# zypher-game/uzkge

Hardware: AMD Instinct MI355X
Metric: bn254_g1_msm_points_per_sec (higher is better)
Workload: dtype u256 (254-bit modular integers: 8 x u32 Montgomery limbs in HBM, 9 x 29-bit limbs in the two hot loops); 1 GPU; BN254 G1 MSM, 2^24 random points + uniform scalars per GPU, bases resident in HBM; points_per_gpu=16777216, total_points=16777216

## Files before the change

### uzkge_amd/csrc/api.cpp

```cpp
#include <algorithm>
#include <atomic>
#include <cstdarg>
#include <cstdlib>
#include <cstring>
#include <exception>
#include <new>

#include "ctx.hpp"
#include "host_ec64.hpp"
#include "host_math.hpp"

namespace uzk {

static thread_local char g_err[512] = "";

void set_error(const char* fmt, ...) {
    va_list ap;
    va_start(ap, fmt);
    vsnprintf(g_err, sizeof g_err, fmt, ap);
    va_end(ap);
}

int on_exception(const char* fn) noexcept {
    try { throw; }
// ... 270 lines not shown
        if (kv.second.owned && kv.second.d_points) (void)hipFree(kv.second.d_points);
        if (kv.second.d_table) (void)hipFree(kv.second.d_table);
    }
    s.srs.clear();
    s.num_cus.clear();
    s.bound = false;
    s.device = -1;
    return UZK_OK;
} catch (...) { return uzk::on_exception("uzk_shutdown"); }

namespace uzk {
static void copy_tuning(const Ctx& from, Ctx& to) {
    to.msm_window_bits = from.msm_window_bits;
    to.tune_no_precompute = from.tune_no_precompute; to.tune_ntt_tile = from.tune_ntt_tile; to.tune_ntt_two_pass = from.tune_ntt_two_pass; to.tune_small = from.tune_small;
    to.tune_chunk_log = from.tune_chunk_log; to.tune_stream_log = from.tune_stream_log; to.tune_stream_min_log = from.tune_stream_min_log;
    to.tune_seg_sort = from.tune_seg_sort; to.tune_arith29 = from.tune_arith29;
}
}
int uzk_ctx_create(uint64_t* ctx_out) try {
    if (!ctx_out) { set_error("uzk_ctx_create: null pointer"); return UZK_ERR_PARAMETER; }
    Ctx* c = new Ctx();
    {
        API_LOCK;
        int rc = require_ready();
        if (rc != UZK_OK) { delete c; return rc; }
        copy_tuning(ctx(), *c);
    }
    Shared& s = shared();
    std::lock_guard<std::mutex> lk(s.mu);
    const uint64_t h = s.next_ctx++;
    s.contexts[h] = c;
// ... 937 lines not shown
    if (!window_bits || !windows || n == 0) { set_error("uzk_msm_plan_info: bad arguments"); return UZK_ERR_PARAMETER; }
    msm_plan_info(ctx(), n, window_bits, windows);
    return UZK_OK;
} catch (...) { return uzk::on_exception("uzk_msm_plan_info"); }

int uzk_tune(const char* key, int value) try {
    API_LOCK;
    if (!key) { set_error("uzk_tune: null key"); return UZK_ERR_PARAMETER; }
    Ctx& c = ctx();
    if (!std::strcmp(key, "msm_no_precompute")) c.tune_no_precompute = value;
    else if (!std::strcmp(key, "msm_stream_log")) c.tune_stream_log = (value >= -1 && value <= 26) ? value : 0;
    else if (!std::strcmp(key, "msm_stream_min_log")) c.tune_stream_min_log = (value >= 4 && value <= 26) ? value : 22;
    else if (!std::strcmp(key, "msm_chunk_log")) c.tune_chunk_log = (value >= 8 && value <= 26) ? value : 26;
    else if (!std::strcmp(key, "msm_small")) c.tune_small = value ? 1 : 0;
    else if (!std::strcmp(key, "msm_seg_sort")) c.tune_seg_sort = value;
    else if (!std::strcmp(key, "ntt_tile")) c.tune_ntt_tile = (value == 1024 || value == 2048) ? value : 0;
    else if (!std::strcmp(key, "ntt_two_pass")) c.tune_ntt_two_pass = value ? 1 : 0;
    else if (!std::strcmp(key, "arith29")) c.tune_arith29 = value & 7;
    else { set_error("uzk_tune: unknown key %s", key); return UZK_ERR_PARAMETER; }
    return UZK_OK;
} catch (...) { return uzk::on_exception("uzk_tune"); }

}
```

### uzkge_amd/csrc/ctx.hpp

```cpp
#pragma once
#include <hip/hip_runtime.h>

#include <cstdint>
#include <cstdlib>
#include <cstdio>
#include <chrono>
#include <map>
#include <mutex>
#include <string>
#include <vector>

#include "../../include/uzkge_gpu.h"
#include "../../include/uzkge_gpu_test.h"
#include "ec.hpp"

namespace uzk {

void set_error(const char* fmt, ...);
int on_exception(const char* fn) noexcept;

#define UZK_HIP(expr)                                                                      \
    do {                                                                                   \
        hipError_t _e = (expr);                                                            \
        if (_e != hipSuccess) {                                                            \
// ... 63 lines not shown
    Fp* msm_tail_host = nullptr;
    size_t msm_tail_cap = 0;
    int msm_window_bits = 0;
    int tune_no_precompute = 0;
    int tune_ntt_two_pass = 1;
    int tune_ntt_tile = 0;
    int tune_small = 1;
    int tune_chunk_log = 26;
    int tune_stream_log = 0;
    int tune_stream_min_log = 22;
    int tune_arith29 = default_arith29();
    static int default_arith29() {
        static const int v = [] { const char* e = std::getenv("UZK_ARITH29"); return e ? std::atoi(e) : 7; }();
        return v;
    }
    int tune_seg_sort = 1;
    DevBuf poly_tmp, poly_tmp2, poly_io, zpoly_tmp, open_tmp, poly_args;
    DevBuf poly_cnt;
    uint32_t trim_flip = 0;
    void* poly_host = nullptr;
    size_t poly_host_cap = 0;
    DevBuf ntt_sub;
    struct PowCache { Fp key; bool valid = false; uint64_t stamp = 0; DevBuf buf; };
    PowCache pow_cache[8];
    uint64_t pow_stamp = 0;
    std::vector<void*> ntt_fused;
    std::map<uint64_t, void*> g1ntt_plans;
    DevBuf g1ntt_work, g1ntt_prefix, g1ntt_io;
    struct Srs {
        Affine* d_points = nullptr;
// ... 151 lines not shown
```

### uzkge_amd/csrc/msm.hip

```cpp
#include <algorithm>
#include <cmath>
#include <mutex>
#include <functional>
#include <memory>
#include <condition_variable>
#include <atomic>
#include <cstring>
#include <thread>
#include <vector>

#include "ctx.hpp"
#include "ec29.hpp"
#include "ecquad.hpp"
#include "ecquad29.hpp"
#include "ec29l.hpp"
#include "host_ec64.hpp"
#include "host_math.hpp"

namespace uzk {

constexpr uint32_t kSeg = 16;
constexpr uint32_t kSignBit = 0x80000000u;
constexpr uint32_t kCombineFan = 32;
constexpr int kMaxPasses = 3;
// ... 485 lines not shown
            }
        }
        __syncthreads();
        if (!direct) {
            const uint32_t hl = tid & 31;
            for (uint32_t b = b_lo + (tid >> 5); b < b_hi; b += TB / 32) {
                const uint32_t c = cnt[b], src = off[b] - base, dst = gdst[b];
                for (uint32_t j = hl; j < c; j += 32) out[dst + j] = buf[src + j];
            }
            __syncthreads();
        }
        b_lo = b_hi;
    }
}

__global__ __launch_bounds__(1024) void msm_scan_win_kernel(const uint32_t* __restrict__ cnt_in, uint32_t div,
                                                            uint32_t* __restrict__ v_out,
                                                            uint32_t* __restrict__ off_out,
                                                            uint32_t* __restrict__ win_total,
                                                            uint32_t* __restrict__ max_out, uint32_t NB,
                                                            uint32_t* __restrict__ len_hist = nullptr) {
    __shared__ uint32_t part[1024];
    __shared__ uint32_t lh[256];
    extern __shared__ uint32_t stage[];
    if (len_hist != nullptr) { if (threadIdx.x < 256) lh[threadIdx.x] = 0; __syncthreads(); }
    const uint32_t w = blockIdx.x, tid = threadIdx.x;
    const uint32_t per = (NB + 1023) / 1024;
    const uint32_t lo = min(NB, tid * per), hi = min(NB, lo + per);
    const uint32_t* cnt = cnt_in + (size_t)w * NB;
    const uint64_t magic = div ? ((1ull << 40) + div - 1) / div : 0;
    const bool fast = div && div <= 1024;
    auto val = [&](uint32_t c) -> uint32_t {
        if (!div) return c;
        if (fast && c < (1u << 29)) return (uint32_t)(((uint64_t)(c + div - 1) * magic) >> 40);
        return (c + div - 1) / div;
    };
    auto pad = [](uint32_t i) -> uint32_t { return i + (i >> 5); };
    uint32_t mx = 0;
    for (uint32_t i = tid; i < NB; i += 1024) {
        const uint32_t c = cnt[i];
        mx = max(mx, c);
        const uint32_t T = val(c);
        stage[pad(i)] = T;
        if (len_hist != nullptr && c != 0) {
            const uint32_t q = c / T, r = c - q * T;
            if (r) atomicAdd(&lh[min(q + 1, 255u)], r);
            atomicAdd(&lh[min(q, 255u)], T - r);
        }
    }
    __syncthreads();
    if (len_hist != nullptr && tid < 256 && lh[tid]) atomicAdd(&len_hist[tid], lh[tid]);
    uint32_t s = 0;
    for (uint32_t b = lo; b < hi; ++b) s += stage[pad(b)];
    part[tid] = s;
    __syncthreads();
    for (uint32_t off = 1; off < 1024; off <<= 1) {
        uint32_t v = (tid >= off) ? part[tid - off] : 0;
        __syncthreads();
        part[tid] += v;
        __syncthreads();
    }
    uint32_t run = part[tid] - s;
    for (uint32_t b = lo; b < hi; ++b) {
        const uint32_t v = stage[pad(b)];
        stage[pad(b)] = run;
        run += v;
    }
    __syncthreads();
    uint32_t* off_o = off_out + (size_t)w * NB;
    uint32_t* v_o = v_out ? v_out + (size_t)w * NB : nullptr;
    for (uint32_t i = tid; i < NB; i += 1024) {
        off_o[i] = stage[pad(i)];
        if (v_o) v_o[i] = val(cnt[i]);
    }
    if (tid == 1023) win_total[w] = part[1023];
    if (max_out) {
        for (int o = 32; o > 0; o >>= 1) mx = max(mx, (uint32_t)__shfl_down((int)mx, o));
        if ((tid & 63) == 0 && mx) atomicMax(max_out, mx);
    }
}
static size_t scan_win_lds(uint32_t NB) {
    static const bool raised = [] {
        return hipFuncSetAttribute(reinterpret_cast<const void*>(msm_scan_win_kernel), hipFuncAttributeMaxDynamicSharedMemorySize,
                                   ((1 << 15) + (1 << 10) + 1) * 4) == hipSuccess;
    }();
    (void)raised;
    return ((size_t)NB + NB / 32 + 1) * 4;
}
__global__ __launch_bounds__(1024) void msm_win_base_kernel(const uint32_t* __restrict__ win_total,
                                                            uint32_t* __restrict__ win_base, uint32_t W) {
    __shared__ uint32_t part[1024];
    const uint32_t tid = threadIdx.x;
    const uint32_t v = tid < W ? win_total[tid] : 0;
// ... 22 lines not shown
        if (win_base[mid] <= tid) lo = mid; else hi = mid;
    }
    w = lo;
    const uint32_t lt = tid - win_base[w];
    const uint32_t* off = task_off + (size_t)w * NB;
    lo = 0; hi = NB;
    while (hi - lo > 1) {
        const uint32_t mid = (lo + hi) >> 1;
        if (off[mid] <= lt) lo = mid; else hi = mid;
    }
    b = lo;
    j = lt - off[lo];
}

struct TaskDesc { uint32_t start, cnt, task; uint32_t pad; };
constexpr uint32_t kLenBins = 256;

__global__ __launch_bounds__(256) void msm_task_scan_kernel(const uint32_t* __restrict__ hist, uint32_t* __restrict__ cursor) {
    __shared__ uint32_t h[kLenBins];
    h[threadIdx.x] = hist[threadIdx.x];
    __syncthreads();
    if (threadIdx.x == 0) {
        uint32_t run = 0;
        for (int l = kLenBins - 1; l >= 0; --l) { const uint32_t v = h[l]; h[l] = run; run += v; }
    }
    __syncthreads();
    cursor[threadIdx.x] = h[threadIdx.x];
}
constexpr uint32_t kFillInline = 4;
struct BigBucket { uint32_t start, total, T, tid0; };
__global__ __launch_bounds__(256) void msm_bucket_fill_kernel(const uint32_t* __restrict__ win_base, const uint32_t* __restrict__ task_cnt,
                                                              const uint32_t* __restrict__ task_off,
                                                              const uint32_t* __restrict__ bucket_start,
                                                              const uint32_t* __restrict__ bucket_count, uint32_t NB, uint64_t TBK,
                                                              uint32_t* __restrict__ cursor, TaskDesc* __restrict__ desc,
                                                              uint32_t* __restrict__ big_count, BigBucket* __restrict__ big, uint32_t direct) {
    __shared__ uint32_t h[kLenBins], base[kLenBins];
    h[threadIdx.x] = 0;
    __syncthreads();
    const uint64_t t = (uint64_t)blockIdx.x * blockDim.x + threadIdx.x;
    uint32_t T = 0, total = 0, q = 0, r = 0, start = 0, tid0 = 0, rank_hi = 0, rank_lo = 0;
    bool inline_fill = false;
    if (t < TBK) {
        T = task_cnt[t];
        if (T != 0) {
            total = bucket_count[t];
            start = bucket_start[t];
            tid0 = win_base[t / NB] + task_off[t];
            q = total / T; r = total - q * T;
            if (T <= kFillInline) {
                inline_fill = true;
                if (r) rank_hi = atomicAdd(&h[min(q + 1, kLenBins - 1)], r);
                rank_lo = atomicAdd(&h[min(q, kLenBins - 1)], T - r);
            } else {
                BigBucket e; e.start = start; e.total = total; e.T = T; e.tid0 = tid0;
                big[atomicAdd(big_count, 1u)] = e;
            }
        }
    }
    __syncthreads();
    if (h[threadIdx.x]) base[threadIdx.x] = atomicAdd(&cursor[threadIdx.x], h[threadIdx.x]);
    __syncthreads();
    if (inline_fill) {
        const uint32_t p_hi = base[min(q + 1, kLenBins - 1)] + rank_hi, p_lo = base[min(q, kLenBins - 1)] + rank_lo;
        for (uint32_t j = 0; j < T; ++j) {
            TaskDesc d;
            d.start = start + j * q + min(j, r);
            d.cnt = q + (j < r ? 1u : 0u);
            d.task = (direct && T == 1) ? (kSignBit | (uint32_t)t) : tid0 + j;
            d.pad = 0;
            desc[j < r ? p_hi + j : p_lo + (j - r)] = d;
        }
    }
}
__global__ __launch_bounds__(64) void msm_task_fill_big_kernel(const uint32_t* __restrict__ big_count, const BigBucket* __restrict__ big,
                                                               uint32_t* __restrict__ cursor, TaskDesc* __restrict__ desc) {
// ... 101 lines not shown
    for (int o = GS / 2; o > 0; o >>= 1) {
        XYZZ q = xyzz_shfl_down(acc, o);
        if (sub + (uint32_t)o < (uint32_t)GS) xyzz_add(acc, q);
    }
    return acc;
}

struct BigFold { uint32_t src, cnt, dst, pad; };
template <int GS>
__global__ __launch_bounds__(256) void msm_combine_kernel(const XYZZ* __restrict__ in, const uint32_t* __restrict__ in_cnt,
                                                          const uint32_t* __restrict__ in_off,
                                                          const uint32_t* __restrict__ in_base,
                                                          const uint32_t* __restrict__ task_off,
                                                          const uint32_t* __restrict__ win_base, XYZZ* __restrict__ out,
                                                          uint32_t NB, uint32_t W, uint32_t G, uint32_t* __restrict__ big_count,
                                                          BigFold* __restrict__ big, uint32_t big_thresh, int arith29) {
    const uint32_t gt = blockIdx.x * blockDim.x + threadIdx.x;
    const uint32_t tid = gt / GS, sub = gt % GS;
    if (tid >= win_base[W]) return;
    uint32_t w, b, j;
    find_task(tid, win_base, W, task_off, NB, w, b, j);
    const uint32_t total = in_cnt[(size_t)w * NB + b];
    const uint32_t first = j * G;
    const uint32_t cnt = min(G, total - first);
    const uint32_t at = in_base[w] + in_off[(size_t)w * NB + b] + first;
    if (GS == 1 && big != nullptr && cnt > big_thresh) {
        BigFold e; e.src = at; e.cnt = cnt; e.dst = tid; e.pad = 0;
        big[atomicAdd(big_count, 1u)] = e;
        return;
    }
    XYZZ acc = arith29 ? fold_partials29<GS>(in + at, cnt, sub) : fold_partials<GS>(in + at, cnt, sub);
    if (sub == 0) out[tid] = acc;
}
__global__ __launch_bounds__(64) void msm_fold_big_kernel(const XYZZ* __restrict__ in, const uint32_t* __restrict__ big_count,
                                                          const BigFold* __restrict__ big, XYZZ* __restrict__ out, int accumulate) {
    const uint32_t total = *big_count, lane = threadIdx.x;
    for (uint32_t i = blockIdx.x; i < total; i += gridDim.x) {
        const BigFold e = big[i];
        XYZZ acc = xyzz_inf();
        for (uint32_t k = lane; k < e.cnt; k += 64) { XYZZ q = in[e.src + k]; xyzz_add(acc, q); }
// ... 2 lines not shown
            if (lane + (uint32_t)o < 64) xyzz_add(acc, q);
        }
        if (lane == 0) {
            if (accumulate) { XYZZ prev = out[e.dst]; xyzz_add(prev, acc); out[e.dst] = prev; }
            else out[e.dst] = acc;
        }
    }
}

template <int GS>
__global__ __launch_bounds__(256) void msm_finalize_kernel(const XYZZ* __restrict__ in, const uint32_t* __restrict__ in_cnt,
                                                           const uint32_t* __restrict__ in_off,
                                                           const uint32_t* __restrict__ in_base,
                                                           XYZZ* __restrict__ buckets, uint32_t NB, uint32_t W, int accumulate,
                                                           uint32_t* __restrict__ big_count, BigFold* __restrict__ big, uint32_t big_thresh,
                                                           int skip_single, int arith29) {
    const size_t gt = (size_t)blockIdx.x * blockDim.x + threadIdx.x;
    const size_t t = gt / GS;
    const uint32_t sub = (uint32_t)(gt % GS);
    if (t >= (size_t)W * NB) return;
    const uint32_t w = (uint32_t)(t / NB);
    const uint32_t cnt = in_cnt[t];
    if (skip_single && cnt == 1) return;
    if (GS == 1 && big != nullptr && cnt > big_thresh) {
        BigFold e; e.src = in_base[w] + in_off[t]; e.cnt = cnt; e.dst = (uint32_t)t; e.pad = 0;
        big[atomicAdd(big_count, 1u)] = e;
        return;
    }
    XYZZ acc = arith29 ? fold_partials29<GS>(in + in_base[w] + in_off[t], cnt, sub) : fold_partials<GS>(in + in_base[w] + in_off[t], cnt, sub);
    if (sub == 0) {
        if (accumulate && cnt != 0) { XYZZ prev = buckets[t]; xyzz_add(prev, acc); buckets[t] = prev; }
        else if (!accumulate) buckets[t] = acc;
    }
}

__global__ __launch_bounds__(256) void msm_undirect_kernel(const XYZZ* __restrict__ buckets, const uint32_t* __restrict__ cnt,
                                                           const uint32_t* __restrict__ off, const uint32_t* __restrict__ base,
                                                           XYZZ* __restrict__ partials, uint32_t NB, uint64_t TBK) {
    const uint64_t t = (uint64_t)blockIdx.x * blockDim.x + threadIdx.x;
    if (t >= TBK || cnt[t] != 1) return;
    partials[base[t / NB] + off[t]] = buckets[t];
}

__global__ __launch_bounds__(256) void msm_reduce_kernel(const XYZZ* __restrict__ buckets, XYZZ* __restrict__ partials,
                                                         uint32_t nbk, uint32_t groups_per_window, uint32_t seg) {
    __shared__ XYZZ sh[256];
    const uint32_t w = blockIdx.y, tid = threadIdx.x;
    const uint32_t g = blockIdx.x * blockDim.x + tid;
// ... 769 lines not shown
struct SortPass { uint32_t shift, bins, nseg, nch, chunk, items_bound; };
constexpr int kSegCfgs = 6;
constexpr uint32_t kSegCap[kSegCfgs] = {128 * 12, 256 * 12, 256 * 24, 256 * 40, 512 * 40, 512 * 72};

struct MsmGroup {
    MsmWork* m = nullptr;
    hipStream_t st = nullptr;
    bool pre = false;
    int cb = 0;
    uint32_t W_total = 0, w0 = 0, W = 0, n32 = 0, batch = 0;
    uint64_t per_poly = 0, entries = 0, TBK = 0, bound0 = 0, part_cap = 0;
    uint32_t kb = 0, NBL = 0, S0 = 0, seg_n = 0, NB = 0, Wd = 0, RW = 0, seg = 0, groups = 0, L = 0;
    int P = 0;
    bool scan_reduce = false, quad_reduce = false;
    bool direct = false;
    uint32_t class_s = 0, nb2 = 0;
    uint32_t rl = 256;
    uint32_t pk_bits = 0;
    SortPass sp[kMaxPasses];
    uint32_t *cnt_cur = nullptr, *off_cur = nullptr, *base_cur = nullptr;
    XYZZ* part_cur = nullptr;
};

static int msm_group_plan(Ctx& c, MsmGroup& g, size_t n, uint32_t batch, int cb, bool pre, uint32_t W_total, uint32_t w0,
                          uint32_t W, uint64_t idx_span = 0) {
    g.pre = pre; g.cb = cb; g.W_total = W_total; g.w0 = w0; g.W = W; g.n32 = (uint32_t)n; g.batch = batch;
    g.per_poly = (uint64_t)W * n;
    g.entries = g.per_poly * batch;
    if (g.entries >= (1ull << 31)) { set_error("msm: batch*W*n overflows the 31-bit index space"); return UZK_ERR_PARAMETER; }
    g.kb = (uint32_t)cb - 1;
// ... 21 lines not shown
        sg = std::max<uint32_t>(1, std::min<uint32_t>(sg, g.NBL / g.rl));
        while ((g.NBL + sg * g.rl - 1) / (sg * g.rl) > g.rl) sg <<= 1;
        g.seg = sg;
    } else {
        g.seg = std::max<uint32_t>(1, std::min<uint32_t>(kSeg, g.NBL / 256));
    }
    g.groups = (g.NBL + g.seg * g.rl - 1) / (g.seg * g.rl);
    g.class_s = 0; g.nb2 = 0;
    if (g.NBL >= 4096 && g.NBL <= (1u << 18) && (uint64_t)g.RW * 2 <= 65535) {
        g.class_s = 8;
        g.nb2 = std::max<uint32_t>(256, g.NBL >> 8);
    }
    const uint64_t all_entries = (uint64_t)W_total * n * batch;
    const uint64_t mean_pop = (pre ? (uint64_t)W_total * n : (uint64_t)n) >> g.kb;
    g.L = (uint32_t)std::max<uint64_t>(16, std::min<uint64_t>(256, std::min<uint64_t>(4 * mean_pop, all_entries / 200000)));
    g.bound0 = g.entries / g.L + g.TBK;
    g.part_cap = g.bound0 + 2 * g.TBK;
    g.P = g.kb <= 9 ? 1 : (g.kb <= 18 ? 2 : 3);
    g.pk_bits = 0;
    if (g.P == 2 && (!pre || idx_span)) {
        uint32_t ib = 1;
        while ((1ull << ib) < (pre ? idx_span : (uint64_t)g.seg_n)) ++ib;
        const uint32_t first_bits = std::min<uint32_t>(9, g.kb - 1);
        if (ib + 1 + (g.kb - first_bits) <= 32) g.pk_bits = ib;
    }
    uint32_t rem = g.kb, nseg = g.S0;
    for (int p = 0; p < g.P; ++p) {
        uint32_t bits = (rem + (uint32_t)(g.P - p) - 1) / (uint32_t)(g.P - p);
        if (g.pk_bits && p == 0) bits = std::min<uint32_t>(9, g.kb - 1);
        rem -= bits;
        g.sp[p].shift = rem;
// ... 17 lines not shown
    if (g.class_s) UZK_TRY(m.class_sums.reserve((size_t)g.RW * 2 * g.nb2 * sizeof(XYZZ)));
    for (int p = 0; p < g.P; ++p) {
        UZK_TRY(m.counts[p].reserve((size_t)(p == 0 ? 2 * g.sp[p].nseg * g.sp[p].nch : g.sp[p].items_bound) * g.sp[p].bins * 4));
        if (p > 0) UZK_TRY(m.items[p].reserve(((size_t)g.sp[p].nseg + 1) * 4));
        if (p + 1 < g.P) {
            UZK_TRY(m.segs_start[p].reserve((size_t)g.sp[p].nseg * g.sp[p].bins * 4));
            UZK_TRY(m.segs_len[p].reserve((size_t)g.sp[p].nseg * g.sp[p].bins * 4));
            UZK_TRY(m.ent[p & 1].reserve((size_t)g.entries * sizeof(uint2)));
        }
    }
    for (int k = 0; k < 2; ++k) {
        UZK_TRY(m.lvl_cnt[k].reserve((size_t)g.TBK * 4));
        UZK_TRY(m.lvl_off[k].reserve((size_t)g.TBK * 4));
    }
    UZK_TRY(m.lvl_part[0].reserve((size_t)g.part_cap * sizeof(XYZZ)));
    UZK_TRY(m.small.reserve(16384));
    UZK_TRY(m.task_desc.reserve((size_t)g.bound0 * sizeof(TaskDesc)));
    UZK_TRY(m.exc.reserve((size_t)g.bound0 * 4));
    if (m.h_sums_cap < (size_t)g.RW * 2) {
        if (m.h_sums) (void)hipHostFree(m.h_sums);
        UZK_HIP(hipHostMalloc(reinterpret_cast<void**>(&m.h_sums), (size_t)g.RW * 2 * sizeof(XYZZ), hipHostMallocDefault));
        m.h_sums_cap = (size_t)g.RW * 2;
    }
    if (!m.h_max) UZK_HIP(hipHostMalloc(reinterpret_cast<void**>(&m.h_max), 64, hipHostMallocDefault));
    return UZK_OK;
}

static int msm_group_phase1(Ctx& c, MsmGroup& g, const Affine* points, const ScalarView& d_scalars, uint32_t pre_stride,
                            uint32_t pre_off, bool direct_ok = true) {
    MsmWork& m = *g.m;
    hipStream_t st = g.st;
    c.cur_stream = st;
    uint32_t* digits = m.digits.as<uint32_t>();
    uint32_t* sorted = m.sorted.as<uint32_t>();
    uint32_t* bcount = m.bucket_count.as<uint32_t>();
    uint32_t* bstart = m.bucket_start.as<uint32_t>();
    uint32_t* sm = m.small.as<uint32_t>();
    uint32_t* win_tot = sm;
    uint32_t* d_max = sm + 3200;
    UZK_HIP(hipMemsetAsync(d_max, 0, (3912 - 3200) * 4, st));
    const bool fused_hist = !g.pre && g.w0 == 0 && g.W == g.W_total && g.sp[0].nch >= 256 &&
                            (size_t)g.W * g.sp[0].bins * 4 <= 64 * 1024;
    if (fused_hist) {
        KernelScope ks(c, "msm_digits");
        hipLaunchKernelGGL(msm_digits_hist_kernel, dim3(g.sp[0].nch, g.batch), dim3(1024), (size_t)g.W * g.sp[0].bins * 4, st,
                           d_scalars, digits, g.n32, g.cb, (int)g.W, g.sp[0].shift, g.sp[0].bins, m.counts[0].as<uint32_t>());
    } else {
        KernelScope ks(c, "msm_digits");
        const uint64_t tot = (uint64_t)g.n32 * g.batch;
        hipLaunchKernelGGL(msm_digits_kernel, dim3((unsigned)((tot + 255) / 256)), dim3(256), 0, st, d_scalars, digits, g.n32,
                           g.batch, g.cb, (int)g.W_total, (int)g.w0, (int)g.W, (uint32_t*)nullptr);
    }
    for (int p = 0; p < g.P; ++p) {
        const bool first = (p == 0), last = (p == g.P - 1);
        const SortPass& sp = g.sp[p];
// ... 75 lines not shown
            if (first && !last && a.pk_out_bits && sp.bins <= 512 && cs0 <= 32768 && !g.pre)
                hipLaunchKernelGGL((msm_radix_chunk_kernel<512, 64, 18176>), grid, dim3(512), 0, st, a);
            else if (first && last) hipLaunchKernelGGL((msm_radix_scatter_kernel<1024, 8, true, true, false>), grid, dim3(1024), 0, st, a);
            else if (first && g.entries >= (1ull << 26))
                hipLaunchKernelGGL((msm_radix_scatter_kernel<512, 8, true, false, false>), grid, dim3(512), 0, st, a);
            else if (first) hipLaunchKernelGGL((msm_radix_scatter_kernel<1024, 8, true, false, false>), grid, dim3(1024), 0, st, a);
            else if (last && a.pk_in_bits) hipLaunchKernelGGL((msm_radix_scatter_kernel<512, 8, false, true, true>), grid, dim3(512), 0, st, a);
            else if (last) hipLaunchKernelGGL((msm_radix_scatter_kernel<256, 16, false, true, false>), grid, dim3(256), 0, st, a);
            else hipLaunchKernelGGL((msm_radix_scatter_kernel<1024, 8, false, false, false>), grid, dim3(1024), 0, st, a);
        }
    }
    g.cnt_cur = m.lvl_cnt[0].as<uint32_t>();
    g.off_cur = m.lvl_off[0].as<uint32_t>();
    g.base_cur = sm + 1024;
    g.part_cur = m.lvl_part[0].as<XYZZ>();
    uint32_t* len_hist = sm + 3328;
    uint32_t* len_cur = sm + 3328 + kLenBins;
    g.direct = direct_ok;
    XYZZ* direct_buckets = g.direct ? m.buckets.as<XYZZ>() : nullptr;
    {
        KernelScope ks(c, "msm_scan_win");
        hipLaunchKernelGGL(msm_scan_win_kernel, dim3(g.Wd), dim3(1024), scan_win_lds(g.NB), st, bcount, g.L, g.cnt_cur, g.off_cur, win_tot,
                           d_max, g.NB, len_hist);
        hipLaunchKernelGGL(msm_win_base_kernel, dim3(1), dim3(1024), 0, st, win_tot, g.base_cur, g.Wd);
    }
    TaskDesc* desc = m.task_desc.as<TaskDesc>();
    {
        KernelScope ks(c, "msm_task_order");
        uint32_t* big_count = sm + 3908;
        UZK_TRY(m.big.reserve((size_t)(g.TBK + 1) * sizeof(BigBucket)));
        hipLaunchKernelGGL(msm_task_scan_kernel, dim3(1), dim3(256), 0, st, len_hist, len_cur);
        hipLaunchKernelGGL(msm_bucket_fill_kernel, dim3((unsigned)((g.TBK + 255) / 256)), dim3(256), 0, st, g.base_cur, g.cnt_cur, g.off_cur,
                           bstart, bcount, g.NB, g.TBK, len_cur, desc, big_count, m.big.as<BigBucket>(), g.direct ? 1u : 0u);
        hipLaunchKernelGGL(msm_task_fill_big_kernel, dim3(1024), dim3(64), 0, st, big_count, m.big.as<BigBucket>(), len_cur, desc);
    }
    {
        KernelScope ks(c, "msm_accumulate");
        const dim3 grid((unsigned)((g.bound0 + 255) / 256));
        uint32_t* exc_count = sm + 3900;
        uint32_t* exc_list = m.exc.as<uint32_t>();
        hipLaunchKernelGGL(msm_accumulate29_kernel, grid, dim3(256), 0, st, points, sorted, desc, g.base_cur, g.part_cur,
                           g.Wd, exc_count, exc_list, direct_buckets);
        hipLaunchKernelGGL(msm_accumulate_exc_kernel, dim3(std::min<unsigned>(grid.x, 128u)), dim3(256), 0, st, points, sorted, desc, g.part_cur,
                           exc_count, exc_list, direct_buckets);
    }
    UZK_HIP(hipGetLastError());
    UZK_HIP(hipMemcpyAsync(m.h_max, d_max, 4, hipMemcpyDeviceToHost, st));
    return UZK_OK;
}

static int msm_group_phase2(Ctx& c, MsmGroup& g, bool accumulate = false, bool reduce = true) {
    const int a29 = (c.tune_arith29 >> 2) & 1;
    MsmWork& m = *g.m;
    hipStream_t st = g.st;
    c.cur_stream = st;
    UZK_HIP(hipStreamSynchronize(st));
    uint32_t* sm = m.small.as<uint32_t>();
    uint32_t* win_tot = sm;
    uint32_t* win_base[2] = {sm + 1024, sm + 2080};
    XYZZ* buckets = m.buckets.as<XYZZ>();
    XYZZ* partials = m.partials.as<XYZZ>();
    XYZZ* win_sums = m.win_sums.as<XYZZ>();
    const uint32_t G = kCombineFan;
    uint64_t tmax = ((uint64_t)m.h_max[0] + g.L - 1) / g.L;
    const uint32_t gs = g.TBK >= (1u << 18) ? 1u : (tmax > 2 ? 4u : 1u);
    constexpr uint32_t kBigThresh = 4;
    static_assert(sizeof(BigFold) == sizeof(BigBucket), "the two lists share one buffer");
    const bool big_mode = gs == 1 && tmax > kBigThresh;
    uint32_t* big_count = sm + 3904;
    BigFold* big_list = nullptr;
    if (big_mode) {
        UZK_TRY(m.big.reserve((size_t)(g.bound0 / G + g.TBK + 1) * sizeof(BigFold)));
        big_list = m.big.as<BigFold>();
    }
    if (g.direct && tmax > G) {
        KernelScope ks(c, "msm_combine");
        hipLaunchKernelGGL(msm_undirect_kernel, dim3((unsigned)((g.TBK + 255) / 256)), dim3(256), 0, st, buckets, g.cnt_cur, g.off_cur,
                           g.base_cur, g.part_cur, g.NB, g.TBK);
        g.direct = false;
    }
    if (accumulate && g.direct) { set_error("msm: direct bucket writes in an accumulating chunk (internal error)"); return UZK_ERR_DEVICE; }
    const int skip_single = g.direct ? 1 : 0;
    int lvl = 0;
    uint64_t bound_prev = g.bound0;
    while (tmax > G) {
        const int nx = (lvl + 1) & 1;
        UZK_TRY(m.lvl_part[nx].reserve((size_t)g.part_cap * sizeof(XYZZ)));
        uint32_t* cnt_nx = m.lvl_cnt[nx].as<uint32_t>();
        uint32_t* off_nx = m.lvl_off[nx].as<uint32_t>();
        uint32_t* base_nx = win_base[nx];
        const uint64_t bound_nx = bound_prev / G + g.TBK;
        XYZZ* part_nx = m.lvl_part[nx].as<XYZZ>();
        {
            KernelScope ks(c, "msm_scan_win");
            hipLaunchKernelGGL(msm_scan_win_kernel, dim3(g.Wd), dim3(1024), scan_win_lds(g.NB), st, g.cnt_cur, G, cnt_nx, off_nx, win_tot,
                               (uint32_t*)nullptr, g.NB);
            hipLaunchKernelGGL(msm_win_base_kernel, dim3(1), dim3(1024), 0, st, win_tot, base_nx, g.Wd);
        }
        {
            KernelScope ks(c, "msm_combine");
            const dim3 grid((unsigned)((bound_nx * gs + 255) / 256));
            if (gs == 16)
                hipLaunchKernelGGL(msm_combine_kernel<16>, grid, dim3(256), 0, st, g.part_cur, g.cnt_cur, g.off_cur, g.base_cur,
                                   off_nx, base_nx, part_nx, g.NB, g.Wd, G, (uint32_t*)nullptr, (BigFold*)nullptr, 0u, a29);
            else if (gs == 4)
                hipLaunchKernelGGL(msm_combine_kernel<4>, grid, dim3(256), 0, st, g.part_cur, g.cnt_cur, g.off_cur, g.base_cur,
                                   off_nx, base_nx, part_nx, g.NB, g.Wd, G, (uint32_t*)nullptr, (BigFold*)nullptr, 0u, a29);
            else {
                if (big_mode) UZK_HIP(hipMemsetAsync(big_count, 0, 4, st));
                hipLaunchKernelGGL(msm_combine_kernel<1>, grid, dim3(256), 0, st, g.part_cur, g.cnt_cur, g.off_cur, g.base_cur,
                                   off_nx, base_nx, part_nx, g.NB, g.Wd, G, big_count, big_list, kBigThresh, a29);
                if (big_mode)
                    hipLaunchKernelGGL(msm_fold_big_kernel, dim3(2048), dim3(64), 0, st, g.part_cur, big_count, big_list, part_nx, 0);
            }
        }
        g.cnt_cur = cnt_nx; g.off_cur = off_nx; g.base_cur = base_nx; g.part_cur = part_nx;
        bound_prev = bound_nx;
        tmax = (tmax + G - 1) / G;
        lvl = nx;
    }
    {
        KernelScope ks(c, "msm_finalize");
        const dim3 grid((unsigned)((g.TBK * gs + 255) / 256));
        if (gs == 16)
            hipLaunchKernelGGL(msm_finalize_kernel<16>, grid, dim3(256), 0, st, g.part_cur, g.cnt_cur, g.off_cur, g.base_cur,
                               buckets, g.NB, g.Wd, accumulate ? 1 : 0, (uint32_t*)nullptr, (BigFold*)nullptr, 0u, skip_single, a29);
        else if (gs == 4)
            hipLaunchKernelGGL(msm_finalize_kernel<4>, grid, dim3(256), 0, st, g.part_cur, g.cnt_cur, g.off_cur, g.base_cur,
                               buckets, g.NB, g.Wd, accumulate ? 1 : 0, (uint32_t*)nullptr, (BigFold*)nullptr, 0u, skip_single, a29);
        else {
            const bool big_last = big_mode && tmax > kBigThresh;
            if (big_last) UZK_HIP(hipMemsetAsync(big_count, 0, 4, st));
            hipLaunchKernelGGL(msm_finalize_kernel<1>, grid, dim3(256), 0, st, g.part_cur, g.cnt_cur, g.off_cur, g.base_cur,
                               buckets, g.NB, g.Wd, accumulate ? 1 : 0, big_count, big_last ? big_list : (BigFold*)nullptr, kBigThresh, skip_single, a29);
            if (big_last)
                hipLaunchKernelGGL(msm_fold_big_kernel, dim3(2048), dim3(64), 0, st, g.part_cur, big_count, big_list, buckets, accumulate ? 1 : 0);
        }
    }
    if (!reduce) { UZK_HIP(hipGetLastError()); return UZK_OK; }
    if (g.class_s) {
        XYZZ* cls = m.class_sums.as<XYZZ>();
        const uint32_t RW2 = g.RW * 2;
        {
            KernelScope ks(c, "msm_reduce_class");
            hipLaunchKernelGGL(msm_class_sums_kernel, dim3(g.NBL / 2048, g.RW, 2), dim3(256), 0, st, buckets, cls, g.NBL, g.class_s, g.nb2, (c.tune_arith29 >> 2) & 1);
        }
        {
            KernelScope ks(c, "msm_reduce");
            const uint32_t seg2 = 4, log_seg2 = 2, groups2 = (g.nb2 + seg2 * kQuadLanes - 1) / (seg2 * kQuadLanes);
            XYZZ* part_r = partials + (size_t)RW2 * groups2;
            hipLaunchKernelGGL(msm_reduce_scan_quad_kernel, dim3(groups2, RW2), dim3(kQuadLanes * 4), 0, st, cls, groups2 == 1 ? win_sums : partials,
                               part_r, g.nb2, groups2, seg2, log_seg2);
// ... 386 lines not shown
```

Before: 867.0 million points/s.

## Split a hashed subset of buckets into shorter tasks to balance the MSM tail

Adds a TaskRule that picks a bit-reversed hash-selected fraction of buckets and splits them into shorter accumulation tasks (len1/len2) while raising the main task length L. The point is to keep the GPU busy during the tail of the bucket-accumulation phase by adding smaller tasks. Those split buckets skip the normal combine/finalize path and are folded by a new msm_fold_steps_kernel. The length histogram grows to 512 bins, and the combine tree now takes the maximum task count directly from the device. The cost is one more kernel launch, more partial-result storage, and extra fold work on the split buckets.

New measurement: 879.8 million points/s (median of 6 runs). 1.01x the previous value.

```diff
diff --git a/uzkge_amd/csrc/api.cpp b/uzkge_amd/csrc/api.cpp
--- a/uzkge_amd/csrc/api.cpp
+++ b/uzkge_amd/csrc/api.cpp
@@ -308,7 +308,7 @@
     to.msm_window_bits = from.msm_window_bits;
     to.tune_no_precompute = from.tune_no_precompute; to.tune_ntt_tile = from.tune_ntt_tile; to.tune_ntt_two_pass = from.tune_ntt_two_pass; to.tune_small = from.tune_small;
     to.tune_chunk_log = from.tune_chunk_log; to.tune_stream_log = from.tune_stream_log; to.tune_stream_min_log = from.tune_stream_min_log;
-    to.tune_seg_sort = from.tune_seg_sort; to.tune_arith29 = from.tune_arith29;
+    to.tune_seg_sort = from.tune_seg_sort; to.tune_arith29 = from.tune_arith29; to.tune_task_tail = from.tune_task_tail;
 }
 }
 int uzk_ctx_create(uint64_t* ctx_out) try {
@@ -1276,6 +1276,11 @@
     else if (!std::strcmp(key, "msm_chunk_log")) c.tune_chunk_log = (value >= 8 && value <= 26) ? value : 26;
     else if (!std::strcmp(key, "msm_small")) c.tune_small = value ? 1 : 0;
     else if (!std::strcmp(key, "msm_seg_sort")) c.tune_seg_sort = value;
+#ifdef UZK_TASK_TAIL_SWEEP
+    else if (!std::strcmp(key, "msm_task_tail")) c.tune_task_tail = value;
+#else
+    else if (!std::strcmp(key, "msm_task_tail")) c.tune_task_tail = (value >= 0 && value <= 2) ? value : 1;
+#endif
     else if (!std::strcmp(key, "ntt_tile")) c.tune_ntt_tile = (value == 1024 || value == 2048) ? value : 0;
     else if (!std::strcmp(key, "ntt_two_pass")) c.tune_ntt_two_pass = value ? 1 : 0;
     else if (!std::strcmp(key, "arith29")) c.tune_arith29 = value & 7;
diff --git a/uzkge_amd/csrc/ctx.hpp b/uzkge_amd/csrc/ctx.hpp
--- a/uzkge_amd/csrc/ctx.hpp
+++ b/uzkge_amd/csrc/ctx.hpp
@@ -101,6 +101,7 @@
         static const int v = [] { const char* e = std::getenv("UZK_ARITH29"); return e ? std::atoi(e) : 7; }();
         return v;
     }
+    int tune_task_tail = 1;
     int tune_seg_sort = 1;
     DevBuf poly_tmp, poly_tmp2, poly_io, zpoly_tmp, open_tmp, poly_args;
     DevBuf poly_cnt;
diff --git a/uzkge_amd/csrc/msm.hip b/uzkge_amd/csrc/msm.hip
--- a/uzkge_amd/csrc/msm.hip
+++ b/uzkge_amd/csrc/msm.hip
@@ -523,42 +523,55 @@
     }
 }
 
-__global__ __launch_bounds__(1024) void msm_scan_win_kernel(const uint32_t* __restrict__ cnt_in, uint32_t div,
+struct TaskRule { uint32_t L, pop_cap, len1, len2, thr1, thr2, shift, split; };
+__device__ __forceinline__ uint32_t task_step_hash(const TaskRule& tr, uint64_t bucket) { return __brev((uint32_t)(bucket >> 6)) >> tr.shift; }
+__device__ __forceinline__ bool task_in_step(const TaskRule& tr, uint64_t bucket) { return tr.thr1 != 0 && task_step_hash(tr, bucket) < tr.thr1; }
+__device__ __forceinline__ uint32_t task_len(const TaskRule& tr, uint64_t bucket, uint32_t pop) {
+    const uint32_t whole = pop <= tr.L ? tr.L : tr.split;
+    if (tr.thr1 == 0 || pop > tr.pop_cap) return whole;
+    const uint32_t h = task_step_hash(tr, bucket);
+    return h < tr.thr2 ? tr.len2 : (h < tr.thr1 ? tr.len1 : whole);
+}
+constexpr uint32_t kLenBins = 512;
+
+__global__ __launch_bounds__(1024) void msm_scan_win_kernel(const uint32_t* __restrict__ cnt_in, TaskRule tr,
                                                             uint32_t* __restrict__ v_out,
                                                             uint32_t* __restrict__ off_out,
                                                             uint32_t* __restrict__ win_total,
                                                             uint32_t* __restrict__ max_out, uint32_t NB,
                                                             uint32_t* __restrict__ len_hist = nullptr) {
     __shared__ uint32_t part[1024];
-    __shared__ uint32_t lh[256];
+    __shared__ uint32_t lh[kLenBins];
     extern __shared__ uint32_t stage[];
-    if (len_hist != nullptr) { if (threadIdx.x < 256) lh[threadIdx.x] = 0; __syncthreads(); }
-    const uint32_t w = blockIdx.x, tid = threadIdx.x;
+    if (len_hist != nullptr) { if (threadIdx.x < kLenBins) lh[threadIdx.x] = 0; __syncthreads(); }
+    const uint32_t w = blockIdx.x, tid = threadIdx.x, div = tr.L;
     const uint32_t per = (NB + 1023) / 1024;
     const uint32_t lo = min(NB, tid * per), hi = min(NB, lo + per);
     const uint32_t* cnt = cnt_in + (size_t)w * NB;
     const uint64_t magic = div ? ((1ull << 40) + div - 1) / div : 0;
     const bool fast = div && div <= 1024;
-    auto val = [&](uint32_t c) -> uint32_t {
+    auto val = [&](uint32_t c, uint32_t i) -> uint32_t {
         if (!div) return c;
+        if (tr.thr1 || tr.split != tr.L) { const uint32_t len = task_len(tr, (uint64_t)w * NB + i, c); return (c + len - 1) / len; }
         if (fast && c < (1u << 29)) return (uint32_t)(((uint64_t)(c + div - 1) * magic) >> 40);
         return (c + div - 1) / div;
     };
     auto pad = [](uint32_t i) -> uint32_t { return i + (i >> 5); };
-    uint32_t mx = 0;
+    uint32_t mx = 0, mt = 0;
     for (uint32_t i = tid; i < NB; i += 1024) {
         const uint32_t c = cnt[i];
         mx = max(mx, c);
-        const uint32_t T = val(c);
+        const uint32_t T = val(c, i);
+        mt = max(mt, T);
         stage[pad(i)] = T;
         if (len_hist != nullptr && c != 0) {
             const uint32_t q = c / T, r = c - q * T;
-            if (r) atomicAdd(&lh[min(q + 1, 255u)], r);
-            atomicAdd(&lh[min(q, 255u)], T - r);
-        }
-    }
-    __syncthreads();
-    if (len_hist != nullptr && tid < 256 && lh[tid]) atomicAdd(&len_hist[tid], lh[tid]);
+            if (r) atomicAdd(&lh[min(q + 1, kLenBins - 1)], r);
+            atomicAdd(&lh[min(q, kLenBins - 1)], T - r);
+        }
+    }
+    __syncthreads();
+    if (len_hist != nullptr && tid < kLenBins && lh[tid]) atomicAdd(&len_hist[tid], lh[tid]);
     uint32_t s = 0;
     for (uint32_t b = lo; b < hi; ++b) s += stage[pad(b)];
     part[tid] = s;
@@ -580,12 +593,15 @@
     uint32_t* v_o = v_out ? v_out + (size_t)w * NB : nullptr;
     for (uint32_t i = tid; i < NB; i += 1024) {
         off_o[i] = stage[pad(i)];
-        if (v_o) v_o[i] = val(cnt[i]);
+        if (v_o) v_o[i] = val(cnt[i], i);
     }
     if (tid == 1023) win_total[w] = part[1023];
     if (max_out) {
-        for (int o = 32; o > 0; o >>= 1) mx = max(mx, (uint32_t)__shfl_down((int)mx, o));
-        if ((tid & 63) == 0 && mx) atomicMax(max_out, mx);
+        for (int o = 32; o > 0; o >>= 1) {
+            mx = max(mx, (uint32_t)__shfl_down((int)mx, o));
+            mt = max(mt, (uint32_t)__shfl_down((int)mt, o));
+        }
+        if ((tid & 63) == 0 && mx) { atomicMax(max_out, mx); atomicMax(max_out + 1, mt); }
     }
 }
 static size_t scan_win_lds(uint32_t NB) {
@@ -638,9 +654,8 @@
 }
 
 struct TaskDesc { uint32_t start, cnt, task; uint32_t pad; };
-constexpr uint32_t kLenBins = 256;
-
-__global__ __launch_bounds__(256) void msm_task_scan_kernel(const uint32_t* __restrict__ hist, uint32_t* __restrict__ cursor) {
+
+__global__ __launch_bounds__(kLenBins) void msm_task_scan_kernel(const uint32_t* __restrict__ hist, uint32_t* __restrict__ cursor) {
     __shared__ uint32_t h[kLenBins];
     h[threadIdx.x] = hist[threadIdx.x];
     __syncthreads();
@@ -651,16 +666,17 @@
     __syncthreads();
     cursor[threadIdx.x] = h[threadIdx.x];
 }
-constexpr uint32_t kFillInline = 4;
+constexpr uint32_t kFillInline = 4, kFillInlineSteps = 64;
 struct BigBucket { uint32_t start, total, T, tid0; };
 __global__ __launch_bounds__(256) void msm_bucket_fill_kernel(const uint32_t* __restrict__ win_base, const uint32_t* __restrict__ task_cnt,
                                                               const uint32_t* __restrict__ task_off,
                                                               const uint32_t* __restrict__ bucket_start,
                                                               const uint32_t* __restrict__ bucket_count, uint32_t NB, uint64_t TBK,
                                                               uint32_t* __restrict__ cursor, TaskDesc* __restrict__ desc,
-                                                              uint32_t* __restrict__ big_count, BigBucket* __restrict__ big, uint32_t direct) {
+                                                              uint32_t* __restrict__ big_count, BigBucket* __restrict__ big, uint32_t direct,
+                                                              uint32_t fill_inline) {
     __shared__ uint32_t h[kLenBins], base[kLenBins];
-    h[threadIdx.x] = 0;
+    for (uint32_t k = threadIdx.x; k < kLenBins; k += blockDim.x) h[k] = 0;
     __syncthreads();
     const uint64_t t = (uint64_t)blockIdx.x * blockDim.x + threadIdx.x;
     uint32_t T = 0, total = 0, q = 0, r = 0, start = 0, tid0 = 0, rank_hi = 0, rank_lo = 0;
@@ -672,7 +688,7 @@
             start = bucket_start[t];
             tid0 = win_base[t / NB] + task_off[t];
             q = total / T; r = total - q * T;
-            if (T <= kFillInline) {
+            if (T <= fill_inline) {
                 inline_fill = true;
                 if (r) rank_hi = atomicAdd(&h[min(q + 1, kLenBins - 1)], r);
                 rank_lo = atomicAdd(&h[min(q, kLenBins - 1)], T - r);
@@ -683,7 +699,8 @@
         }
     }
     __syncthreads();
-    if (h[threadIdx.x]) base[threadIdx.x] = atomicAdd(&cursor[threadIdx.x], h[threadIdx.x]);
+    for (uint32_t k = threadIdx.x; k < kLenBins; k += blockDim.x)
+        if (h[k]) base[k] = atomicAdd(&cursor[k], h[k]);
     __syncthreads();
     if (inline_fill) {
         const uint32_t p_hi = base[min(q + 1, kLenBins - 1)] + rank_hi, p_lo = base[min(q, kLenBins - 1)] + rank_lo;
@@ -815,7 +832,7 @@
                                                           const uint32_t* __restrict__ task_off,
                                                           const uint32_t* __restrict__ win_base, XYZZ* __restrict__ out,
                                                           uint32_t NB, uint32_t W, uint32_t G, uint32_t* __restrict__ big_count,
-                                                          BigFold* __restrict__ big, uint32_t big_thresh, int arith29) {
+                                                          BigFold* __restrict__ big, uint32_t big_thresh, int arith29, TaskRule steps) {
     const uint32_t gt = blockIdx.x * blockDim.x + threadIdx.x;
     const uint32_t tid = gt / GS, sub = gt % GS;
     if (tid >= win_base[W]) return;
@@ -825,6 +842,7 @@
     const uint32_t first = j * G;
     const uint32_t cnt = min(G, total - first);
     const uint32_t at = in_base[w] + in_off[(size_t)w * NB + b] + first;
+    if (total <= G && task_in_step(steps, (uint64_t)w * NB + b)) return;
     if (GS == 1 && big != nullptr && cnt > big_thresh) {
         BigFold e; e.src = at; e.cnt = cnt; e.dst = tid; e.pad = 0;
         big[atomicAdd(big_count, 1u)] = e;
@@ -857,12 +875,13 @@
                                                            const uint32_t* __restrict__ in_base,
                                                            XYZZ* __restrict__ buckets, uint32_t NB, uint32_t W, int accumulate,
                                                            uint32_t* __restrict__ big_count, BigFold* __restrict__ big, uint32_t big_thresh,
-                                                           int skip_single, int arith29) {
+                                                           int skip_single, int arith29, TaskRule steps) {
     const size_t gt = (size_t)blockIdx.x * blockDim.x + threadIdx.x;
     const size_t t = gt / GS;
     const uint32_t sub = (uint32_t)(gt % GS);
     if (t >= (size_t)W * NB) return;
     const uint32_t w = (uint32_t)(t / NB);
+    if (task_in_step(steps, t)) return;
     const uint32_t cnt = in_cnt[t];
     if (skip_single && cnt == 1) return;
     if (GS == 1 && big != nullptr && cnt > big_thresh) {
@@ -875,6 +894,28 @@
         if (accumulate && cnt != 0) { XYZZ prev = buckets[t]; xyzz_add(prev, acc); buckets[t] = prev; }
         else if (!accumulate) buckets[t] = acc;
     }
+}
+
+struct FoldStepsArgs {
+    const XYZZ* in; const uint32_t *in_cnt, *in_off, *in_base;
+    XYZZ* out; const uint32_t *out_off, *out_base;
+    uint32_t NB, G; uint64_t TBK; TaskRule steps; int accumulate, skip_single, arith29;
+};
+__global__ __launch_bounds__(256) void msm_fold_steps_kernel(FoldStepsArgs a) {
+    const uint64_t o = (uint64_t)blockIdx.x * blockDim.x + threadIdx.x;
+    const uint64_t grp = o >> 6;
+    const uint32_t i = (uint32_t)(grp % a.steps.thr1);
+    const uint64_t g = ((grp / a.steps.thr1) << (32 - a.steps.shift)) | (__brev(i) >> a.steps.shift);
+    const uint64_t t = g * 64 + (o & 63);
+    if (t >= a.TBK) return;
+    const uint32_t w = (uint32_t)(t / a.NB);
+    const uint32_t cnt = a.in_cnt[t];
+    if (a.out_off != nullptr ? (cnt == 0 || cnt > a.G) : (a.skip_single && cnt == 1)) return;
+    const XYZZ* src = a.in + a.in_base[w] + a.in_off[t];
+    XYZZ acc = a.arith29 ? fold_partials29<1>(src, cnt, 0) : fold_partials<1>(src, cnt, 0);
+    if (a.out_off != nullptr) a.out[a.out_base[w] + a.out_off[t]] = acc;
+    else if (a.accumulate && cnt != 0) { XYZZ prev = a.out[t]; xyzz_add(prev, acc); a.out[t] = prev; }
+    else if (!a.accumulate) a.out[t] = acc;
 }
 
 __global__ __launch_bounds__(256) void msm_undirect_kernel(const XYZZ* __restrict__ buckets, const uint32_t* __restrict__ cnt,
@@ -1674,6 +1715,7 @@
     int P = 0;
     bool scan_reduce = false, quad_reduce = false;
     bool direct = false;
+    TaskRule rule{};
     uint32_t class_s = 0, nb2 = 0;
     uint32_t rl = 256;
     uint32_t pk_bits = 0;
@@ -1725,7 +1767,52 @@
     const uint64_t all_entries = (uint64_t)W_total * n * batch;
     const uint64_t mean_pop = (pre ? (uint64_t)W_total * n : (uint64_t)n) >> g.kb;
     g.L = (uint32_t)std::max<uint64_t>(16, std::min<uint64_t>(256, std::min<uint64_t>(4 * mean_pop, all_entries / 200000)));
-    g.bound0 = g.entries / g.L + g.TBK;
+    g.rule = TaskRule{g.L, 0, 0, 0, 0, 0, 16, g.L};
+    uint64_t step_tasks = 0;
+    {
+        constexpr uint32_t kTailMinRes = 3, kTailLenFloor = 8;
+        uint32_t res1_q = 8, res2_q = 4, len_cap = kLenBins - 1, div1 = 4, div2 = 8;
+#ifdef UZK_TASK_TAIL_SWEEP
+        if (c.tune_task_tail >= 16) {
+            const uint32_t v = (uint32_t)c.tune_task_tail;
+            res1_q = (v >> 4) & 63; res2_q = (v >> 10) & 63; len_cap = std::min<uint32_t>(kLenBins - 1, ((v >> 16) & 127) * 8);
+            div1 = (v >> 23) & 15; div2 = ((v >> 27) & 15) * 4;
+        }
+#endif
+        const int mode = c.tune_task_tail & 15;
+        const uint64_t resident = (uint64_t)std::max(1, c.num_cus) * 4 * 4 * 64;
+        const uint64_t typical = std::max<uint64_t>(1, std::min<uint64_t>(g.L, mean_pop));
+        bool take = mode == 1 && g.entries / typical >= kTailMinRes * resident && mean_pop >= g.L;
+#ifdef UZK_TASK_TAIL_SWEEP
+        if (c.tune_task_tail >= 16) take = mode == 1 && g.entries / typical >= kTailMinRes * resident && typical >= 4 * kTailLenFloor;
+#endif
+        if (mode == 2 || take) {
+            TaskRule r{};
+            r.split = g.L;
+            r.L = (uint32_t)std::max<uint64_t>(g.L, std::min<uint64_t>(len_cap, std::min<uint64_t>(4 * mean_pop, all_entries / 200000)));
+            r.len1 = div1 ? std::max<uint32_t>(kTailLenFloor, (uint32_t)typical / div1) : 0;
+            r.len2 = div2 ? std::max<uint32_t>(kTailLenFloor, (uint32_t)typical / div2) : 0;
+            if (r.len1 == 0 || r.len2 >= r.len1) { r.len1 = std::max(r.len1, r.len2); r.len2 = 0; res1_q = r.len1 ? std::max(res1_q, res2_q) : 0; }
+            const uint64_t groups = (g.TBK + 63) / 64;
+            uint32_t bits = 4;
+            while (bits < 16 && (1ull << bits) < groups) ++bits;
+            r.shift = 32 - bits;
+            auto share = [&](uint32_t res_q, uint32_t len) -> uint32_t {
+                return len ? (uint32_t)std::min<uint64_t>((1u << bits) / 4, ((res_q * resident * len / 4) << bits) / std::max<uint64_t>(1, g.entries)) : 0u;
+            };
+            r.thr2 = share(res2_q, r.len2);
+            r.thr1 = r.thr2 + share(res1_q, r.len1);
+            r.pop_cap = std::min<uint32_t>(r.L, kCombineFan * (r.len2 ? r.len2 : std::max(1u, r.len1)));
+            if (r.thr1) {
+                const uint64_t blocks = (groups + (1ull << bits) - 1) >> bits;
+                const uint64_t n2 = std::min<uint64_t>(g.TBK, blocks * r.thr2 * 64), n1 = std::min<uint64_t>(g.TBK, blocks * (r.thr1 - r.thr2) * 64);
+                step_tasks = n1 * ((r.pop_cap + r.len1 - 1) / r.len1) + (r.thr2 ? n2 * ((r.pop_cap + r.len2 - 1) / r.len2) : 0);
+            }
+            g.L = r.L;
+            g.rule = r;
+        }
+    }
+    g.bound0 = g.entries / g.rule.split + g.TBK + step_tasks;
     g.part_cap = g.bound0 + 2 * g.TBK;
     g.P = g.kb <= 9 ? 1 : (g.kb <= 18 ? 2 : 3);
     g.pk_bits = 0;
@@ -1773,7 +1860,7 @@
         UZK_TRY(m.lvl_off[k].reserve((size_t)g.TBK * 4));
     }
     UZK_TRY(m.lvl_part[0].reserve((size_t)g.part_cap * sizeof(XYZZ)));
-    UZK_TRY(m.small.reserve(16384));
+    UZK_TRY(m.small.reserve(32768));
     UZK_TRY(m.task_desc.reserve((size_t)g.bound0 * sizeof(TaskDesc)));
     UZK_TRY(m.exc.reserve((size_t)g.bound0 * 4));
     if (m.h_sums_cap < (size_t)g.RW * 2) {
@@ -1797,7 +1884,8 @@
     uint32_t* sm = m.small.as<uint32_t>();
     uint32_t* win_tot = sm;
     uint32_t* d_max = sm + 3200;
-    UZK_HIP(hipMemsetAsync(d_max, 0, (3912 - 3200) * 4, st));
+    static_assert(4096 + 2 * kLenBins <= 32768 / 4, "the schedule's counters lie inside MsmWork::small");
+    UZK_HIP(hipMemsetAsync(d_max, 0, (4096 + 2 * kLenBins - 3200) * 4, st));
     const bool fused_hist = !g.pre && g.w0 == 0 && g.W == g.W_total && g.sp[0].nch >= 256 &&
                             (size_t)g.W * g.sp[0].bins * 4 <= 64 * 1024;
     if (fused_hist) {
@@ -1903,13 +1991,18 @@
     g.off_cur = m.lvl_off[0].as<uint32_t>();
     g.base_cur = sm + 1024;
     g.part_cur = m.lvl_part[0].as<XYZZ>();
-    uint32_t* len_hist = sm + 3328;
-    uint32_t* len_cur = sm + 3328 + kLenBins;
+    uint32_t* len_hist = sm + 4096;
+    uint32_t* len_cur = sm + 4096 + kLenBins;
     g.direct = direct_ok;
     XYZZ* direct_buckets = g.direct ? m.buckets.as<XYZZ>() : nullptr;
+    if (g.rule.L != g.L || m.small.cap < (4096 + 2 * kLenBins) * 4 || m.task_desc.cap < (size_t)g.bound0 * sizeof(TaskDesc) ||
+        m.exc.cap < (size_t)g.bound0 * 4 || m.lvl_part[0].cap < (size_t)g.part_cap * sizeof(XYZZ) || g.part_cap < g.bound0 + 2 * g.TBK) {
+        set_error("msm: task schedule: a workspace is smaller than its launch needs (internal error)");
+        return UZK_ERR_DEVICE;
+    }
     {
         KernelScope ks(c, "msm_scan_win");
-        hipLaunchKernelGGL(msm_scan_win_kernel, dim3(g.Wd), dim3(1024), scan_win_lds(g.NB), st, bcount, g.L, g.cnt_cur, g.off_cur, win_tot,
+        hipLaunchKernelGGL(msm_scan_win_kernel, dim3(g.Wd), dim3(1024), scan_win_lds(g.NB), st, bcount, g.rule, g.cnt_cur, g.off_cur, win_tot,
                            d_max, g.NB, len_hist);
         hipLaunchKernelGGL(msm_win_base_kernel, dim3(1), dim3(1024), 0, st, win_tot, g.base_cur, g.Wd);
     }
@@ -1918,9 +2011,10 @@
         KernelScope ks(c, "msm_task_order");
         uint32_t* big_count = sm + 3908;
         UZK_TRY(m.big.reserve((size_t)(g.TBK + 1) * sizeof(BigBucket)));
-        hipLaunchKernelGGL(msm_task_scan_kernel, dim3(1), dim3(256), 0, st, len_hist, len_cur);
+        hipLaunchKernelGGL(msm_task_scan_kernel, dim3(1), dim3(kLenBins), 0, st, len_hist, len_cur);
         hipLaunchKernelGGL(msm_bucket_fill_kernel, dim3((unsigned)((g.TBK + 255) / 256)), dim3(256), 0, st, g.base_cur, g.cnt_cur, g.off_cur,
-                           bstart, bcount, g.NB, g.TBK, len_cur, desc, big_count, m.big.as<BigBucket>(), g.direct ? 1u : 0u);
+                           bstart, bcount, g.NB, g.TBK, len_cur, desc, big_count, m.big.as<BigBucket>(), g.direct ? 1u : 0u,
+                           g.rule.thr1 ? kFillInlineSteps : kFillInline);
         hipLaunchKernelGGL(msm_task_fill_big_kernel, dim3(1024), dim3(64), 0, st, big_count, m.big.as<BigBucket>(), len_cur, desc);
     }
     {
@@ -1934,7 +2028,7 @@
                            exc_count, exc_list, direct_buckets);
     }
     UZK_HIP(hipGetLastError());
-    UZK_HIP(hipMemcpyAsync(m.h_max, d_max, 4, hipMemcpyDeviceToHost, st));
+    UZK_HIP(hipMemcpyAsync(m.h_max, d_max, 8, hipMemcpyDeviceToHost, st));
     return UZK_OK;
 }
 
@@ -1951,7 +2045,7 @@
     XYZZ* partials = m.partials.as<XYZZ>();
     XYZZ* win_sums = m.win_sums.as<XYZZ>();
     const uint32_t G = kCombineFan;
-    uint64_t tmax = ((uint64_t)m.h_max[0] + g.L - 1) / g.L;
+    uint64_t tmax = m.h_max[1];
     const uint32_t gs = g.TBK >= (1u << 18) ? 1u : (tmax > 2 ? 4u : 1u);
     constexpr uint32_t kBigThresh = 4;
     static_assert(sizeof(BigFold) == sizeof(BigBucket), "the two lists share one buffer");
@@ -1972,6 +2066,14 @@
     const int skip_single = g.direct ? 1 : 0;
     int lvl = 0;
     uint64_t bound_prev = g.bound0;
+    TaskRule steps = g.rule;
+    if (gs != 1) steps.thr1 = 0;
+    auto fold_steps = [&](XYZZ* out, const uint32_t* out_off, const uint32_t* out_base) {
+        if (!steps.thr1) return;
+        const uint64_t blocks = (((g.TBK + 63) / 64) + (1ull << (32 - steps.shift)) - 1) >> (32 - steps.shift);
+        const FoldStepsArgs a{g.part_cur, g.cnt_cur, g.off_cur, g.base_cur, out, out_off, out_base, g.NB, G, g.TBK, steps, accumulate ? 1 : 0, skip_single, a29};
+        hipLaunchKernelGGL(msm_fold_steps_kernel, dim3((unsigned)((blocks * steps.thr1 * 64 + 255) / 256)), dim3(256), 0, st, a);
+    };
     while (tmax > G) {
         const int nx = (lvl + 1) & 1;
         UZK_TRY(m.lvl_part[nx].reserve((size_t)g.part_cap * sizeof(XYZZ)));
@@ -1982,7 +2084,7 @@
         XYZZ* part_nx = m.lvl_part[nx].as<XYZZ>();
         {
             KernelScope ks(c, "msm_scan_win");
-            hipLaunchKernelGGL(msm_scan_win_kernel, dim3(g.Wd), dim3(1024), scan_win_lds(g.NB), st, g.cnt_cur, G, cnt_nx, off_nx, win_tot,
+            hipLaunchKernelGGL(msm_scan_win_kernel, dim3(g.Wd), dim3(1024), scan_win_lds(g.NB), st, g.cnt_cur, TaskRule{G, 0, 0, 0, 0, 0, 16, G}, cnt_nx, off_nx, win_tot,
                                (uint32_t*)nullptr, g.NB);
             hipLaunchKernelGGL(msm_win_base_kernel, dim3(1), dim3(1024), 0, st, win_tot, base_nx, g.Wd);
         }
@@ -1991,20 +2093,22 @@
             const dim3 grid((unsigned)((bound_nx * gs + 255) / 256));
             if (gs == 16)
                 hipLaunchKernelGGL(msm_combine_kernel<16>, grid, dim3(256), 0, st, g.part_cur, g.cnt_cur, g.off_cur, g.base_cur,
-                                   off_nx, base_nx, part_nx, g.NB, g.Wd, G, (uint32_t*)nullptr, (BigFold*)nullptr, 0u, a29);
+                                   off_nx, base_nx, part_nx, g.NB, g.Wd, G, (uint32_t*)nullptr, (BigFold*)nullptr, 0u, a29, steps);
             else if (gs == 4)
                 hipLaunchKernelGGL(msm_combine_kernel<4>, grid, dim3(256), 0, st, g.part_cur, g.cnt_cur, g.off_cur, g.base_cur,
-                                   off_nx, base_nx, part_nx, g.NB, g.Wd, G, (uint32_t*)nullptr, (BigFold*)nullptr, 0u, a29);
+                                   off_nx, base_nx, part_nx, g.NB, g.Wd, G, (uint32_t*)nullptr, (BigFold*)nullptr, 0u, a29, steps);
             else {
                 if (big_mode) UZK_HIP(hipMemsetAsync(big_count, 0, 4, st));
                 hipLaunchKernelGGL(msm_combine_kernel<1>, grid, dim3(256), 0, st, g.part_cur, g.cnt_cur, g.off_cur, g.base_cur,
-                                   off_nx, base_nx, part_nx, g.NB, g.Wd, G, big_count, big_list, kBigThresh, a29);
+                                   off_nx, base_nx, part_nx, g.NB, g.Wd, G, big_count, big_list, kBigThresh, a29, steps);
                 if (big_mode)
                     hipLaunchKernelGGL(msm_fold_big_kernel, dim3(2048), dim3(64), 0, st, g.part_cur, big_count, big_list, part_nx, 0);
             }
+            fold_steps(part_nx, off_nx, base_nx);
         }
         g.cnt_cur = cnt_nx; g.off_cur = off_nx; g.base_cur = base_nx; g.part_cur = part_nx;
         bound_prev = bound_nx;
+        steps.thr1 = 0;
         tmax = (tmax + G - 1) / G;
         lvl = nx;
     }
@@ -2013,18 +2117,19 @@
         const dim3 grid((unsigned)((g.TBK * gs + 255) / 256));
         if (gs == 16)
             hipLaunchKernelGGL(msm_finalize_kernel<16>, grid, dim3(256), 0, st, g.part_cur, g.cnt_cur, g.off_cur, g.base_cur,
-                               buckets, g.NB, g.Wd, accumulate ? 1 : 0, (uint32_t*)nullptr, (BigFold*)nullptr, 0u, skip_single, a29);
+                               buckets, g.NB, g.Wd, accumulate ? 1 : 0, (uint32_t*)nullptr, (BigFold*)nullptr, 0u, skip_single, a29, steps);
         else if (gs == 4)
             hipLaunchKernelGGL(msm_finalize_kernel<4>, grid, dim3(256), 0, st, g.part_cur, g.cnt_cur, g.off_cur, g.base_cur,
-                               buckets, g.NB, g.Wd, accumulate ? 1 : 0, (uint32_t*)nullptr, (BigFold*)nullptr, 0u, skip_single, a29);
+                               buckets, g.NB, g.Wd, accumulate ? 1 : 0, (uint32_t*)nullptr, (BigFold*)nullptr, 0u, skip_single, a29, steps);
         else {
             const bool big_last = big_mode && tmax > kBigThresh;
             if (big_last) UZK_HIP(hipMemsetAsync(big_count, 0, 4, st));
             hipLaunchKernelGGL(msm_finalize_kernel<1>, grid, dim3(256), 0, st, g.part_cur, g.cnt_cur, g.off_cur, g.base_cur,
-                               buckets, g.NB, g.Wd, accumulate ? 1 : 0, big_count, big_last ? big_list : (BigFold*)nullptr, kBigThresh, skip_single, a29);
+                               buckets, g.NB, g.Wd, accumulate ? 1 : 0, big_count, big_last ? big_list : (BigFold*)nullptr, kBigThresh, skip_single, a29, steps);
             if (big_last)
                 hipLaunchKernelGGL(msm_fold_big_kernel, dim3(2048), dim3(64), 0, st, g.part_cur, big_count, big_list, buckets, accumulate ? 1 : 0);
         }
+        fold_steps(buckets, nullptr, nullptr);
     }
     if (!reduce) { UZK_HIP(hipGetLastError()); return UZK_OK; }
     if (g.class_s) {
```
